# scorbiclife/LifeAPI

Hardware: AMD Instinct MI355X
Metric: 64x64 universe-generations/sec (+ cell-updates/sec) at 1/2/4/8 MI355X (higher is better)
Workload: dtype u64

## Files before the change

lifeapi_amd/csrc/cone_passes.hpp:

```cpp
#pragma once

#include "cone_window.hpp"
#include "life_gen.hpp"

namespace lifeapi_impl {
namespace {

template <int P, int UPW, int RMAX, bool FIRST, typename OutT, bool PIPE = false>
__device__ __forceinline__ void cone_wave(const uint64_t *in, const uint64_t *__restrict__ wanted,
                                          const uint64_t *__restrict__ unwanted, OutT *__restrict__ out,
                                          uint64_t n, uint64_t u_first, uint64_t u_step, uint32_t gens,
                                          uint32_t xs, uint32_t K, int lane) {
  constexpr int GPS = kWave / P;
  static_assert(UPW % GPS == 0, "a wave takes whole register sets");
  constexpr int R = UPW / GPS;
  constexpr int RB = R < RMAX ? R : RMAX;
  static_assert(R % RB == 0, "passes of RB sets");
  const uint32_t j = (uint32_t)lane & (P - 1), q = (uint32_t)lane / P;
  const uint32_t col = (xs + j) & (kWave - 1);
  const bool live = j < K;
  const uint64_t w64 = live ? wanted[col] : 0ull, m64 = live ? (w64 | unwanted[col]) : 0ull;
  const W tw = split(w64), tm = split(m64);
  const uint32_t sh = q * P;
  auto clean = [&](W s) __attribute__((always_inline)) {
    const uint32_t d = ((s.lo ^ tw.lo) & tm.lo) | ((s.hi ^ tw.hi) & tm.hi);
    const uint64_t bad = __ballot(d != 0u);
    if constexpr (P == kWave) return bad == 0ull;
    else return ((bad >> sh) & ((1ull << P) - 1)) == 0ull;
  };
  static_assert(UPW <= kWave, "one result per lane");
  for (uint64_t u0 = u_first; u0 < n; u0 += u_step) {
    uint32_t mine = 0;
    auto load = [&](int pass, W (&a)[RB]) __attribute__((always_inline)) {
      const uint64_t ub = u0 + (uint64_t)pass * RB * GPS + q;
#pragma unroll
      for (int k = 0; k < RB; ++k) {
        const uint64_t u = ub + (uint64_t)k * GPS;
        a[k] = (live && u < n) ? ld<true>(in + u * kWave + col) : W{0u, 0u};
      }
    };
    W nx[RB];
    if constexpr (PIPE) load(0, nx);
#pragma unroll 1
    for (int pass = 0; pass < R / RB; ++pass) {
      W a[RB];
      if constexpr (PIPE) {
#pragma unroll
        for (int k = 0; k < RB; ++k) a[k] = nx[k];
        if (pass + 1 < R / RB) load(pass + 1, nx);
      } else {
        load(pass, a);
      }
      uint32_t res[RB];
      if constexpr (FIRST) {
#pragma unroll
        for (int k = 0; k < RB; ++k) res[k] = 0;
        for (uint32_t g = 1; g <= gens; ++g) {
#pragma unroll
          for (int k = 0; k < RB; ++k) {
            a[k] = life_gen<XDPP, 3>(a[k], nullptr, lane);
            if (res[k] == 0 && clean(a[k])) res[k] = g;
          }
        }
      } else {
#pragma unroll
        for (int k = 0; k < RB; ++k) res[k] = clean(a[k]) ? 1u : 0u;
      }
#pragma unroll
      for (int k = 0; k < RB; ++k) {
        const uint32_t first = (uint32_t)(pass * RB + k) * GPS, rel = (uint32_t)lane - first;
        uint32_t v = res[k];
        if constexpr (GPS > 1) v = (uint32_t)__shfl((int)v, (int)((rel & (GPS - 1)) * P));
        if (rel < (uint32_t)GPS) mine = v;
      }
    }
    if (lane < UPW && u0 + lane < n) out[u0 + lane] = (OutT)mine;
  }
}

template <int P, int UPW, int RMAX, int PK, bool WRAP, typename OutT>
__device__ __forceinline__ void cone_wave_rows(const uint64_t *in, const uint64_t *__restrict__ wanted,
                                               const uint64_t *__restrict__ unwanted, OutT *__restrict__ out,
                                               uint64_t n, uint64_t u_first, uint64_t u_step, uint32_t gens,
                                               uint32_t xs, uint32_t K, uint32_t y0, int lane) {
  constexpr int GPS = kWave / P, FW = 32 / PK, UPR = GPS * PK;
  static_assert(PK == 1 || PK == 2 || PK == 4, "fields of 32, 16 or 8 rows");
  static_assert(UPW % UPR == 0 && UPW <= kWave, "a wave takes whole registers, one result per lane");
  constexpr int R = UPW / UPR;
  constexpr int RB = R < RMAX ? R : RMAX;
  static_assert(R % RB == 0, "passes of RB registers");
  constexpr uint32_t fmask = FW == 32 ? ~0u : (1u << FW) - 1u;
  constexpr uint32_t rep = PK == 1 ? 1u : PK == 2 ? 0x00010001u : 0x01010101u;
  constexpr uint32_t kDiff = ((TA ^ TB) & TC) & 0xFF;
  const uint32_t j = (uint32_t)lane & (P - 1), q = (uint32_t)lane / P;
  const uint32_t col = (xs + j) & (kWave - 1);
  const bool live = j < K;
  const uint32_t sh = y0 & 31u, gsh = q * P;
  auto cut = [&](uint64_t v) __attribute__((always_inline)) {
    const W w = split(v);
    return WRAP ? __builtin_amdgcn_alignbit(w.lo, w.hi, sh) : __builtin_amdgcn_alignbit(w.hi, w.lo, sh);
  };
  const uint64_t w64 = live ? wanted[col] : 0ull, m64 = live ? (w64 | unwanted[col]) : 0ull;
  const uint32_t tw = (cut(w64) & fmask) * rep, tm = (cut(m64) & fmask) * rep;
  for (uint64_t u0 = u_first; u0 < n; u0 += u_step) {
    uint32_t mine = 0;
#pragma unroll 1
    for (int pass = 0; pass < R / RB; ++pass) {
      const uint64_t ub = u0 + (uint64_t)pass * RB * UPR + q;
      uint32_t a[RB];
#pragma unroll
      for (int k = 0; k < RB; ++k) {
        uint32_t e[PK];
#pragma unroll
        for (int f = 0; f < PK; ++f) {
          const uint64_t u = ub + (uint64_t)(k * UPR + f * GPS);
          e[f] = (live && u < n) ? cut(__builtin_nontemporal_load(in + u * kWave + col)) : 0u;
        }
        if constexpr (PK == 1) {
          a[k] = e[0];
        } else if constexpr (PK == 2) {
          a[k] = __builtin_amdgcn_perm(e[1], e[0], 0x05040100u);
        } else {
          const uint32_t p01 = __builtin_amdgcn_perm(e[1], e[0], 0x0C0C0400u);
          const uint32_t p23 = __builtin_amdgcn_perm(e[3], e[2], 0x0C0C0400u);
          a[k] = __builtin_amdgcn_perm(p23, p01, 0x05040100u);
        }
      }
      uint32_t res[RB][PK];
#pragma unroll
      for (int k = 0; k < RB; ++k)
#pragma unroll
        for (int f = 0; f < PK; ++f) res[k][f] = 0;
      for (uint32_t g = 1; g <= gens; ++g) {
#pragma unroll
        for (int k = 0; k < RB; ++k) {
          const uint32_t L = dpp_prev(a[k]), Rt = dpp_next(a[k]);
          const uint32_t h0 = lut3<kXor3>(L, a[k], Rt), h1 = lut3<kMaj>(L, a[k], Rt);
          a[k] = life_tail6(h0 << 1, h0, h0 >> 1, h1 << 1, h1, h1 >> 1, a[k]);
          const uint32_t d = lut3<kDiff>(a[k], tw, tm);
#pragma unroll
          for (int f = 0; f < PK; ++f) {
            const uint64_t bad = __ballot((d & (fmask << (f * FW))) != 0u);
            bool clean;
            if constexpr (P == kWave) clean = bad == 0ull;
            else clean = ((bad >> gsh) & ((1ull << P) - 1)) == 0ull;
            if (res[k][f] == 0 && clean) res[k][f] = g;
          }
        }
      }
#pragma unroll
      for (int k = 0; k < RB; ++k)
#pragma unroll
        for (int f = 0; f < PK; ++f) {
          const uint32_t first = (uint32_t)((pass * RB + k) * UPR + f * GPS), rel = (uint32_t)lane - first;
          uint32_t v = res[k][f];
          if constexpr (GPS > 1) v = (uint32_t)__shfl((int)v, (int)((rel & (GPS - 1)) * P));
          if (rel < (uint32_t)GPS) mine = v;
        }
    }
    if (lane < UPW && u0 + lane < n) out[u0 + lane] = (OutT)mine;
  }
}

template <int UPW, int RMAX>
__device__ __forceinline__ void cone_wave_full16(const uint64_t *in, const uint64_t *__restrict__ wanted,
                                                 const uint64_t *__restrict__ unwanted, uint8_t *__restrict__ out,
                                                 uint64_t n, uint64_t u_first, uint64_t u_step, int lane) {
  constexpr int RB = UPW / 2 < RMAX ? UPW / 2 : RMAX;
  static_assert(UPW % (2 * RB) == 0, "passes of 2 RB universes");
  const int half = lane >> 5, col = (lane & 31) * 2;
  const uint64_t w0 = wanted[col], w1 = wanted[col + 1];
  const uint64_t m0 = w0 | unwanted[col], m1 = w1 | unwanted[col + 1];
  for (uint64_t u0 = u_first; u0 < n; u0 += u_step) {
    uint32_t mine = 0;
#pragma unroll 1
    for (int pass = 0; pass < UPW / (2 * RB); ++pass) {
      const uint64_t ub = u0 + (uint64_t)pass * 2 * RB;
      u64x2 v[RB];
#pragma unroll
      for (int k = 0; k < RB; ++k) {
        const uint64_t u = ub + 2 * k + half;
        v[k] = u < n ? __builtin_nontemporal_load(reinterpret_cast<const u64x2 *>(in + u * kWave + col))
                     : u64x2{w0, w1};
      }
#pragma unroll
      for (int k = 0; k < RB; ++k) {
        const uint64_t d = ((v[k][0] ^ w0) & m0) | ((v[k][1] ^ w1) & m1);
        const uint64_t bad = __ballot(d != 0ull);
        const uint32_t rel = (uint32_t)lane - (uint32_t)(pass * 2 * RB + 2 * k);
        if (rel < 2u) mine = (uint32_t)(bad >> (32 * rel)) == 0u ? 1u : 0u;
      }
    }
    if (lane < UPW && u0 + lane < n) out[u0 + lane] = (uint8_t)mine;
  }
}

template <int RB>
__device__ __forceinline__ void dma_fetch_pass(const uint64_t *in, uint64_t n, uint64_t ub, int lane, uint64_t *img) {
#pragma unroll
  for (int i = 0; i < RB / 2; ++i) {
    uint64_t u = ub + 2 * i + (lane >> 5);
    if (u >= n) u = n - 1;
    const char *src = reinterpret_cast<const char *>(in + u * kWave) + (lane & 31) * 16;
    __builtin_amdgcn_global_load_lds((const __attribute__((address_space(1))) void *)src,
                                     (__attribute__((address_space(3))) void *)(img + i * 2 * kWave), 16, 0, 2);
  }
}

template <int RB, bool FIRST, typename OutT>
__device__ __forceinline__ void cone_wave_full_dma(const uint64_t *in, uint64_t w64, uint64_t m64,
                                                   OutT *__restrict__ out, uint64_t n, uint64_t u_first,
                                                   uint64_t u_step, uint32_t gens, int lane, uint64_t *img,
                                                   bool prefetched) {
  static_assert(RB % 2 == 0 && 2 * RB <= kWave, "passes of pairs of universes, one answer per lane");
  const W tw = split(w64), tm = split(m64);
  auto clean = [&](W s) __attribute__((always_inline)) {
    const uint32_t d = ((s.lo ^ tw.lo) & tm.lo) | ((s.hi ^ tw.hi) & tm.hi);
    return __ballot(d != 0u) == 0ull;
  };
  auto base = [&](uint64_t t) { return u_first + (t >> 1) * u_step + (t & 1) * RB; };
  auto fetch = [&](uint64_t ub) __attribute__((always_inline)) { dma_fetch_pass<RB>(in, n, ub, lane, img); };
  if (u_first >= n) return;
  if (!prefetched) fetch(u_first);
  uint32_t mine = 0;
  int after = 0;
  for (uint64_t t = 0;; ++t) {
    const uint64_t ub = base(t);
    if (ub >= n) break;
    if (after) __builtin_amdgcn_s_waitcnt(kWaitVm1);
    else __builtin_amdgcn_s_waitcnt(kWaitVm0);
    W a[RB];
#pragma unroll
    for (int k = 0; k < RB; ++k) a[k] = split(img[k * kWave + lane]);
    __builtin_amdgcn_s_waitcnt(kWaitLgkm0);
    const uint64_t nb = base(t + 1);
    if (nb < n) fetch(nb);
    uint32_t res[RB];
    if constexpr (FIRST) {
#pragma unroll
      for (int k = 0; k < RB; ++k) res[k] = 0;
      for (uint32_t g = 1; g <= gens; ++g) {
#pragma unroll
        for (int k = 0; k < RB; ++k) {
          a[k] = life_gen<XDPP, 3>(a[k], nullptr, lane);
          if (res[k] == 0 && clean(a[k])) res[k] = g;
        }
      }
    } else {
#pragma unroll
      for (int k = 0; k < RB; ++k) res[k] = clean(a[k]) ? 1u : 0u;
    }
#pragma unroll
    for (int k = 0; k < RB; ++k)
      if ((uint32_t)lane == (uint32_t)((t & 1) * RB + k)) mine = res[k];
    after = 0;
    if ((t & 1) || ub + RB >= n) {
      const uint64_t u0 = base(t & ~1ull);
      if (lane < 2 * RB && u0 + lane < n) out[u0 + lane] = (OutT)mine;
      mine = 0;
      after = 1;
    }
  }
}

template <int RB, int PK, bool WRAP, typename OutT, int SLEEP = 0>
__device__ __forceinline__ void cone_wave_rows_dma(const uint64_t *in, uint64_t w64, uint64_t m64,
                                                   OutT *__restrict__ out, uint64_t n, uint64_t u_first,
                                                   uint64_t u_step, uint32_t gens, uint32_t y0, int lane,
                                                   uint64_t *img, bool prefetched) {
  static_assert(RB % 2 == 0 && RB % PK == 0 && 2 * RB <= kWave, "passes of whole words and pairs of universes");
  static_assert(PK == 1 || PK == 2 || PK == 4, "fields of 32, 16 or 8 rows");
  constexpr int FW = 32 / PK, NW = RB / PK;
  constexpr uint32_t fmask = FW == 32 ? ~0u : (1u << FW) - 1u;
  constexpr uint32_t rep = PK == 1 ? 1u : PK == 2 ? 0x00010001u : 0x01010101u;
  const uint32_t sh = y0 & 31u;
  auto cut = [&](uint64_t v) __attribute__((always_inline)) {
    const W w = split(v);
    return WRAP ? __builtin_amdgcn_alignbit(w.lo, w.hi, sh) : __builtin_amdgcn_alignbit(w.hi, w.lo, sh);
  };
  const uint32_t tw = (cut(w64) & fmask) * rep, tm = (cut(m64) & fmask) * rep;
  constexpr uint32_t kDiff = ((TA ^ TB) & TC) & 0xFF;
  auto base = [&](uint64_t t) { return u_first + (t >> 1) * u_step + (t & 1) * RB; };
  auto fetch = [&](uint64_t ub) __attribute__((always_inline)) { dma_fetch_pass<RB>(in, n, ub, lane, img); };
  if (u_first >= n) return;
  if (!prefetched) fetch(u_first);
  uint32_t mine = 0;
  int after = 0;
  for (uint64_t t = 0;; ++t) {
    const uint64_t ub = base(t);
    if (ub >= n) break;
    if (after) __builtin_amdgcn_s_waitcnt(kWaitVm1);
    else __builtin_amdgcn_s_waitcnt(kWaitVm0);
    uint32_t a[NW];
#pragma unroll
    for (int m = 0; m < NW; ++m) {
      uint32_t e[PK];
#pragma unroll
      for (int j = 0; j < PK; ++j) e[j] = cut(img[(m * PK + j) * kWave + lane]);
      if constexpr (PK == 1) {
        a[m] = e[0];
      } else if constexpr (PK == 2) {
        a[m] = __builtin_amdgcn_perm(e[1], e[0], 0x05040100u);
      } else {
        const uint32_t p01 = __builtin_amdgcn_perm(e[1], e[0], 0x0C0C0400u);
        const uint32_t p23 = __builtin_amdgcn_perm(e[3], e[2], 0x0C0C0400u);
        a[m] = __builtin_amdgcn_perm(p23, p01, 0x05040100u);
      }
    }
    __builtin_amdgcn_s_waitcnt(kWaitLgkm0);
    const uint64_t nb = base(t + 1);
    if (nb < n) fetch(nb);
    if constexpr (SLEEP > 0) __builtin_amdgcn_s_sleep(SLEEP);
    uint32_t res[RB];
#pragma unroll
    for (int k = 0; k < RB; ++k) res[k] = 0;
    for (uint32_t g = 1; g <= gens; ++g) {
#pragma unroll
      for (int m = 0; m < NW; ++m) {
        const uint32_t L = dpp_prev(a[m]), R = dpp_next(a[m]);
        const uint32_t h0 = lut3<kXor3>(L, a[m], R), h1 = lut3<kMaj>(L, a[m], R);
        a[m] = life_tail6(h0 << 1, h0, h0 >> 1, h1 << 1, h1, h1 >> 1, a[m]);
        const uint32_t d = lut3<kDiff>(a[m], tw, tm);
#pragma unroll
        for (int j = 0; j < PK; ++j) {
          const bool clean = __ballot((d & (fmask << (j * FW))) != 0u) == 0ull;
          if (res[m * PK + j] == 0 && clean) res[m * PK + j] = g;
        }
      }
    }
#pragma unroll
    for (int k = 0; k < RB; ++k)
      if ((uint32_t)lane == (uint32_t)((t & 1) * RB + k)) mine = res[k];
    after = 0;
    if ((t & 1) || ub + RB >= n) {
      const uint64_t u0 = base(t & ~1ull);
      if (lane < 2 * RB && u0 + lane < n) out[u0 + lane] = (OutT)mine;
      mine = 0;
      after = 1;
    }
  }
}

}
}
```

Measured before the change: 7.242 billion.

## Interleave life generations in pairs and pack clean flags into a lane bitmask

Replaces the per-universe life_gen calls with a grouped generation step that evaluates two universes' DPP shifts and LUT stages side by side, with a scheduling barrier after each group, to expose instruction-level parallelism. Per-universe result tracking is replaced by a bitmask of clean flags that each lane indexes directly, which removes the per-k compare/select chains and the res array. A whole-pass DMA fetch that uses instruction offsets is added for small RB when the pass lies fully in range. The grouping raises register pressure, and the sched barriers may constrain the compiler's scheduling.

New measurement: 7.218 billion. No clear change (-0.3%).

```diff
diff --git a/lifeapi_amd/csrc/cone_passes.hpp b/lifeapi_amd/csrc/cone_passes.hpp
--- a/lifeapi_amd/csrc/cone_passes.hpp
+++ b/lifeapi_amd/csrc/cone_passes.hpp
@@ -207,19 +207,69 @@
   }
 }
 
+template <int RB, int I = 0>
+__device__ __forceinline__ void dma_fetch_whole(const char *src, uint64_t *img) {
+  static_assert(RB / 2 * 1024 <= 4096, "the instruction offset is 12 bits");
+  if constexpr (I < RB / 2) {
+    __builtin_amdgcn_global_load_lds((const __attribute__((address_space(1))) void *)src,
+                                     (__attribute__((address_space(3))) void *)img, 16, I * 1024, 2);
+    dma_fetch_whole<RB, I + 1>(src, img);
+  }
+}
+
+template <int N>
+__device__ __forceinline__ void life_gen_group(W *x) {
+  W L[N], R[N], h0[N], h1[N], h0u[N], h0d[N], h1u[N], h1d[N];
+#pragma unroll
+  for (int i = 0; i < N; ++i) L[i] = W{dpp_prev(x[i].lo), dpp_prev(x[i].hi)};
+#pragma unroll
+  for (int i = 0; i < N; ++i) R[i] = W{dpp_next(x[i].lo), dpp_next(x[i].hi)};
+#pragma unroll
+  for (int i = 0; i < N; ++i) h0[i] = lut3<kXor3>(L[i], x[i], R[i]);
+#pragma unroll
+  for (int i = 0; i < N; ++i) h1[i] = lut3<kMaj>(L[i], x[i], R[i]);
+#pragma unroll
+  for (int i = 0; i < N; ++i) h0u[i] = rot_up(h0[i]), h0d[i] = rot_dn(h0[i]);
+#pragma unroll
+  for (int i = 0; i < N; ++i) h1u[i] = rot_up(h1[i]), h1d[i] = rot_dn(h1[i]);
+  uint32_t g1[2 * N], g2[2 * N], g3[2 * N], g4[2 * N], g5[2 * N];
+#define LIFEAPI_HALF(a, j) ((j) & 1 ? a[(j) >> 1].hi : a[(j) >> 1].lo)
+#pragma unroll
+  for (int j = 0; j < 2 * N; ++j) g1[j] = lut3<kN1>(LIFEAPI_HALF(h1, j), LIFEAPI_HALF(h1u, j), LIFEAPI_HALF(h1d, j));
+#pragma unroll
+  for (int j = 0; j < 2 * N; ++j) g2[j] = lut3<kMaj>(LIFEAPI_HALF(h1d, j), LIFEAPI_HALF(h1u, j), LIFEAPI_HALF(h0d, j));
+#pragma unroll
+  for (int j = 0; j < 2 * N; ++j) g3[j] = lut3<kNae>(LIFEAPI_HALF(h0d, j), LIFEAPI_HALF(h0u, j), LIFEAPI_HALF(h0, j));
+#pragma unroll
+  for (int j = 0; j < 2 * N; ++j) g4[j] = lut3<kN4>(g3[j], g2[j], g1[j]);
+#pragma unroll
+  for (int j = 0; j < 2 * N; ++j) g5[j] = lut3<kXor3>(LIFEAPI_HALF(h0, j), LIFEAPI_HALF(h0d, j), LIFEAPI_HALF(h0u, j));
+#pragma unroll
+  for (int i = 0; i < N; ++i)
+    x[i] = W{lut3<kN6>(g4[2 * i], g5[2 * i], x[i].lo), lut3<kN6>(g4[2 * i + 1], g5[2 * i + 1], x[i].hi)};
+#undef LIFEAPI_HALF
+}
+
 template <int RB, bool FIRST, typename OutT>
 __device__ __forceinline__ void cone_wave_full_dma(const uint64_t *in, uint64_t w64, uint64_t m64,
                                                    OutT *__restrict__ out, uint64_t n, uint64_t u_first,
                                                    uint64_t u_step, uint32_t gens, int lane, uint64_t *img,
                                                    bool prefetched) {
-  static_assert(RB % 2 == 0 && 2 * RB <= kWave, "passes of pairs of universes, one answer per lane");
+  static_assert(RB % 2 == 0 && 2 * RB <= kWave && RB <= 32, "passes of pairs of universes, one answer per lane");
+  constexpr int kGroup = 2;
   const W tw = split(w64), tm = split(m64);
-  auto clean = [&](W s) __attribute__((always_inline)) {
+  auto miss = [&](W s) __attribute__((always_inline)) {
     const uint32_t d = ((s.lo ^ tw.lo) & tm.lo) | ((s.hi ^ tw.hi) & tm.hi);
-    return __ballot(d != 0u) == 0ull;
+    return __ballot(d != 0u);
   };
   auto base = [&](uint64_t t) { return u_first + (t >> 1) * u_step + (t & 1) * RB; };
-  auto fetch = [&](uint64_t ub) __attribute__((always_inline)) { dma_fetch_pass<RB>(in, n, ub, lane, img); };
+  auto fetch = [&](uint64_t ub) __attribute__((always_inline)) {
+    if constexpr (RB <= 8) {
+      if (ub + RB <= n)
+        return dma_fetch_whole<RB>(reinterpret_cast<const char *>(in + ub * kWave) + (uint32_t)lane * 16u, img);
+    }
+    dma_fetch_pass<RB>(in, n, ub, lane, img);
+  };
   if (u_first >= n) return;
   if (!prefetched) fetch(u_first);
   uint32_t mine = 0;
@@ -235,24 +285,30 @@
     __builtin_amdgcn_s_waitcnt(kWaitLgkm0);
     const uint64_t nb = base(t + 1);
     if (nb < n) fetch(nb);
-    uint32_t res[RB];
+    const uint32_t rel = (uint32_t)lane - (uint32_t)(t & 1) * RB;
+    uint32_t r = 0;
     if constexpr (FIRST) {
-#pragma unroll
-      for (int k = 0; k < RB; ++k) res[k] = 0;
       for (uint32_t g = 1; g <= gens; ++g) {
-#pragma unroll
-        for (int k = 0; k < RB; ++k) {
-          a[k] = life_gen<XDPP, 3>(a[k], nullptr, lane);
-          if (res[k] == 0 && clean(a[k])) res[k] = g;
-        }
+        uint64_t bad[RB];
+#pragma unroll
+        for (int k = 0; k < RB; k += kGroup) {
+          life_gen_group<kGroup>(a + k);
+#pragma unroll
+          for (int i = 0; i < kGroup; ++i) bad[k + i] = miss(a[k + i]);
+          __builtin_amdgcn_sched_barrier(0);
+        }
+        uint32_t cm = 0;
+#pragma unroll
+        for (int k = 0; k < RB; ++k) cm |= (bad[k] == 0ull ? 1u : 0u) << k;
+        r = (r == 0u) & ((cm >> (rel & 31u)) & 1u) ? g : r;
       }
     } else {
-#pragma unroll
-      for (int k = 0; k < RB; ++k) res[k] = clean(a[k]) ? 1u : 0u;
-    }
-#pragma unroll
-    for (int k = 0; k < RB; ++k)
-      if ((uint32_t)lane == (uint32_t)((t & 1) * RB + k)) mine = res[k];
+      uint32_t cm = 0;
+#pragma unroll
+      for (int k = 0; k < RB; ++k) cm |= (miss(a[k]) == 0ull ? 1u : 0u) << k;
+      r = (cm >> (rel & 31u)) & 1u;
+    }
+    if (rel < (uint32_t)RB) mine = r;
     after = 0;
     if ((t & 1) || ub + RB >= n) {
       const uint64_t u0 = base(t & ~1ull);
```
